# YiyanXu/DiFashion

Measured on AMD Instinct MI355X. Metric: U-Net denoise steps/sec, 4-item outfit @ 64x64x4 latent, higher is better.
Workload: dtype bf16; 1 GPU; BASELINE configs[1]: one 4-item outfit, CFG on (4 branches) -> U-Net batch 16, DDIM-50 schedule, sd15 shape in_channels=8, 64x64x4 latents, 77 text tokens; one outfit per GPU; unet_batch=16, latent=64x64x4, parallelism=outfit-replicas x1 (no data-path collective)

## Files before the change

difashion_amd/csrc/gemm.h:

```cpp
#pragma once
#include <stdint.h>
#include "dfh_common.h"

enum GemmAct { ACT_NONE = 0, ACT_SILU = 1, ACT_LEAKY = 2, ACT_TANH = 3, ACT_GEGLU = 4 };
enum GemmOut {
  OUT_BF16 = 0,
  OUT_BF16_T = 1,
  OUT_F32 = 2,
  OUT_F32_T = 3,
  OUT_FP8_MX = 4,
};

struct GemmArgs {
  const bf16_t* conv_src; int conv_c; int ntaps;
  int Hin, Win, Hout, Wout, stride, ups;
  int pad0;
  const bf16_t* p_src[2]; int p_c[2]; int nplain;
  const bf16_t* W; int ldw;
  const bf16_t* zero;
  int M, N;
  int ksteps;
  int ksplit;
  int n_major;
  int tm_xm, tm_gm;
// ... 21 lines not shown
  const uint8_t* sx;
  const uint8_t* W; const float* sW;
  int M, N, K;
  const float* bias;
  const bf16_t* resid; int ld_res;
  int act;
  void* out; int ld_out; int out_mode;
  uint8_t* out_sx;
  int rows_per_b;
  float* amax;
  const uint8_t* zero;
};

#ifdef __HIPCC__
DFH_DEVICE float2 ln_row_stats(const GemmArgs& a, int m) {
  if (m >= a.M) return float2{0.f, 1.f};
  float sm = 0.f, sq = 0.f, s2 = 0.f;
  for (int t = 0; t < a.ln_parts; ++t) {
    const float2 r = *(const float2*)(a.ln_stat + ((long)t * a.M + m) * 2);
    sm += r.x; sq = fmaf(r.x, r.x, sq); s2 += r.y;
  }
  const float inv = 1.0f / (float)a.ln_parts;
  const float mean = sm * inv;
  const float m2 = s2 + (float)a.ln_cnt * fmaxf(sq - sm * mean, 0.f);
  const float var = m2 * inv / (float)a.ln_cnt;
  return float2{mean, rsqrtf(var + a.ln_eps)};
}
#endif

namespace dfh {
int gemm_fp8_launch(Fp8GemmArgs a, hipStream_t stream);
int amax_slabs_launch(const bf16_t* x, long bstride, int ld, int cols, const int* row0, const int* nrows, float* out, int nslab, int B,
                      hipStream_t stream);
int quant_rows_fp8_launch(const bf16_t* x, int ldx, uint8_t* q, float* scale, int R, int K, hipStream_t stream);
int layernorm_fp8_launch(const bf16_t* x, const float* gamma, const float* beta, uint8_t* q, float* scale, int M, int C, float eps,
                         hipStream_t stream);
int gemm_launch(GemmArgs a, hipStream_t stream, int force_tile = 0, int force_split = 0, int force_order = -1,
                int* gstat_rows = nullptr,
                int* rowstat_bn = nullptr);
int ln_fold_launch(const bf16_t* W, int ldw, const float* gamma, const float* beta, const float* bias, bf16_t* WF, float* s, float* b,
                   int N, int K, hipStream_t stream);
int wino_weight_launch(const bf16_t* W, int ldw, bf16_t* U, int N, int C, int blocked, hipStream_t stream);
bool wino_blocked(int N, int C);
int wino_input_launch(const bf16_t* g, bf16_t* V, int B, int H, int W, int C, hipStream_t stream);
bool gn_wino_ok(int C0, int C1, int G, int H, int W);
int gn_wino_input_launch(const bf16_t* src0, int C0, const bf16_t* src1, int C1, const float* gamma, const float* beta, float eps, int G,
                         bf16_t* V, int B, int H, int W, hipStream_t stream, const bf16_t* Mprev = nullptr, const float* pbias = nullptr,
                         const float* prowvec = nullptr, int prv_ld = 0, int prv_off = 0);
int wino_output_launch(const bf16_t* Mb, bf16_t* out, const float* bias, const float* rowvec, int rv_ld, int rv_off, const bf16_t* resid,
                       int B, int H, int W, int N, hipStream_t stream);
int wino_gemm_tile(const GemmArgs& a);
int ups_phase_fold_launch(const bf16_t* W, int ldw, bf16_t* WP, int N, int C, hipStream_t stream);
int matvec_bias_launch(const bf16_t* W, int ldw, const float* v, const float* b_add, float* b_out, int N, int K, hipStream_t stream);
bool gemm_out2_ok(GemmArgs a);
bool gemm_ln_consumer_ok(GemmArgs a);
int gemm_pick_split(const GemmArgs& a, int* tile_out);
size_t gemm_partial_floats(const GemmArgs& a);
int gemm_count_ksteps(const GemmArgs& a);
bool gemm_wide_eligible(const GemmArgs& a);
int gemm_wide_pick(const GemmArgs& a);
int gemm_wide_launch(GemmArgs a, hipStream_t stream, int variant = 1);
#ifdef DFH_PROBES
bool gemm_halo_eligible(const GemmArgs& a);
int gemm_halo_launch(GemmArgs a, hipStream_t stream);
int gemm_ws_pick(const GemmArgs& a, int min_tiles);
int gemm_ws_launch(GemmArgs a, hipStream_t stream, int bn);
bool gemm_geglu_rows_ok(const GemmArgs& a);
int gemm_geglu_rows_launch(const GemmArgs& a, hipStream_t stream);
bool gemm_persist_ok(const GemmArgs& a);
int gemm_persist_launch(const GemmArgs& a, hipStream_t stream, int max_wgs = 0);
#endif
}
```

difashion_amd/csrc/gemm.hip:

```cpp
#include "gemm.h"
#include "gemm_kiter.h"
#include "gemm_wide_epilogue.h"
#include "norm.h"
#ifdef DFH_PROBES
#include "token_linear.h"
#endif

#include <algorithm>
#include <cstdlib>
#include <cstring>
#include <string>

namespace {

template <int N> DFH_DEVICE void wait_vmcnt() { asm volatile("s_waitcnt vmcnt(%0)" ::"n"(N) : "memory"); }

template <int BM, int BN, int WM, int WN, int NSTAGE, bool LEAN = false, bool WEPI = false>
__global__ __launch_bounds__(WM* WN * 64, (WM * WN == 8 && BM == 128 && 2 * NSTAGE * (BM + BN) * BK * 2 <= 160 * 1024) ? 4 : (WM * WN == 8 ? 2 : 1))
void gemm_bf16_kernel(const GemmArgs a) {
  constexpr int NWV = WM * WN;
  constexpr int TM = BM / WM, TN = BN / WN;
  constexpr int FM = TM / 16, FN = TN / 16;
  constexpr int PA = BM / 8, PB = BN / 8;
  constexpr int IA = (PA + NWV - 1) / NWV, IB = (PB + NWV - 1) / NWV;
// ... 756 lines not shown
  double kk = (double)a.ntaps * a.conv_c;
  for (int i = 0; i < a.nplain; ++i) kk += a.p_c[i];
  const double w_bytes = (double)a.N * kk * 2.0;
  const double a_bytes = a.ntaps ? (double)(a.M / (a.Hout * a.Wout)) * a.Hin * a.Win * a.conv_c * 2.0 : (double)a.M * kk * 2.0;
  const int ntm = (a.M + bm - 1) / bm, ntn = (a.N + bn - 1) / bn;
  if (w_bytes <= 2.0e6 || ntm < 16) return;
  if (ntn >= 16) { a.tm_gm = 8; return; }
  if (!a.ntaps) return;
  int best = 8; double cost = a_bytes + 8.0 * w_bytes;
  for (int xm = 4; xm >= 2; xm >>= 1) {
    if (ntm % xm || ntn % (8 / xm)) continue;
    const double c = (8.0 / xm) * a_bytes + xm * w_bytes;
    if (c < 0.95 * cost) { cost = c; best = xm; }
  }
  if (best != 8) { a.tm_xm = best; a.tm_gm = 8; }
}

int gemm_big_pick(const GemmArgs& a) {
  static const int mode = [] { const char* e = getenv("DFH_GEMM_BIG"); return e ? atoi(e) : 2; }();
  if (mode == 0) return 0;
  if (a.out_mode != OUT_BF16 || a.act == ACT_GEGLU || a.ln_stat) return 0;
  if (a.N % 320 != 0 || (a.ld_out & 7) || (a.resid && (a.ld_res & 7))) return 0;
  const int ksteps = gemm_count_ksteps(a);
  if (ksteps < 16 && (a.ntaps || mode < 3)) return 0;
  if (a.ntaps == 0 && mode < 2) return 0;
  const long tiles = (long)((a.M + 255) / 256) * (a.N / 320), rem = tiles % 256;
  return (tiles >= 224 && (rem == 0 || rem >= 224 || tiles >= 1024)) ? 1 : 0;
}

int gemm_big_geglu_pick(const GemmArgs& a) {
  static const int mode = [] { const char* e = getenv("DFH_GEMM_BIGG"); return e ? atoi(e) : 1; }();
  if (mode == 0 || a.act != ACT_GEGLU || a.out_mode != OUT_BF16 || a.resid || a.rowvec) return 0;
  if (a.N % 256 != 0 || (a.ld_out & 7)) return 0;
  const long tiles = (long)((a.M + 255) / 256) * (a.N / 256), rem = tiles % 256;
  return (tiles >= 224 && (rem == 0 || rem >= 224 || tiles >= 512)) ? 1 : 0;
}

bool wino_blocked(int N, int C) {
  static const bool off = [] { const char* e = getenv("DFH_W_BLOCKED"); return e && e[0] == '0'; }();
  return !off && N % 160 == 0 && C % 64 == 0;
}

int wino_gemm_tile(const GemmArgs& a) {
  static const int pin = [] { const char* e = getenv("DFH_WINO_TILE"); return e ? atoi(e) : -1; }();
  if (pin >= 0) return pin;
  return 0;
}

static bool batched_big_pick(const GemmArgs& a) {
  static const bool off = [] { const char* e = getenv("DFH_BATCH_BIG"); return e && e[0] == '0'; }();
  if (off || a.nbatch <= 1 || a.M < 512 || a.N % 320 != 0) return false;
  const long tiles = (long)((a.M + 255) / 256) * (a.N / 320) * a.nbatch, rem = tiles % 256;
  return tiles >= 224 && (rem == 0 || rem >= 224 || tiles >= 1024);
}

bool gemm_out2_ok(GemmArgs a) {
  if (a.rows_per_b <= 0) a.rows_per_b = a.M;
  a.ksteps = gemm_count_ksteps(a);
  int tile;
  if (gemm_pick_split(a, &tile) != 1) return false;
  return a.out2 != nullptr && a.n_split > 0 && a.n_split < a.N && a.n_split % kTiles[tile].bn == 0 && a.act != ACT_GEGLU &&
         a.out_mode == OUT_BF16 && !a.resid;
}

bool gemm_ln_consumer_ok(GemmArgs a) {
  if (a.rows_per_b <= 0) a.rows_per_b = a.M;
  a.ksteps = gemm_count_ksteps(a);
  int tile;
  if (gemm_pick_split(a, &tile) != 1) return false;
  if (a.act == ACT_GEGLU && ((a.ld_out & 7) || a.N % 32)) return false;
  return a.ntaps == 0 && a.resid == nullptr && a.rowvec == nullptr;
}

int gemm_launch(GemmArgs a, hipStream_t stream, int force_tile, int force_split, int force_order, int* gstat_rows, int* rowstat_bn) {
  if (gstat_rows) *gstat_rows = 0;
  if (rowstat_bn) *rowstat_bn = 0;
  DFH_REQUIRE(a.M > 0 && a.N > 0, "empty GEMM");
  DFH_REQUIRE(a.N % 4 == 0, "N must be a multiple of 4");
  DFH_REQUIRE(a.ntaps == 0 || a.ntaps == 9 || (a.ntaps == 4 && a.phase2x), "ntaps must be 0 or 9 (4 for the phase planes of an upsample conv)");
  DFH_REQUIRE(a.ntaps + a.nplain >= 1, "no K segment");
  DFH_REQUIRE(a.ntaps == 0 || a.conv_c % 8 == 0, "conv channels must be a multiple of 8");
  for (int i = 0; i < a.nplain; ++i) DFH_REQUIRE(a.p_c[i] % 8 == 0, "segment length must be a multiple of 8");
  DFH_REQUIRE(a.zero != nullptr, "zero page missing");
  if (a.rows_per_b <= 0) a.rows_per_b = a.M;
#ifdef DFH_PROBES
  if (force_tile == 30) {
    if (rowstat_bn && a.rowstat) *rowstat_bn = a.N;
    return token_linear_from_gemm(a, stream);
  }
#endif
  a.ksteps = gemm_count_ksteps(a);
  int tile;
  int split = gemm_pick_split(a, &tile);
  const bool force_deep = force_tile == 10;
  if (force_deep) { tile = kEightWave; force_tile = 0; }
  int force_wide = force_tile > kNumTiles ? force_tile - kNumTiles : 0;
  if (force_wide) force_tile = 0;
  if (force_tile > 0) { DFH_REQUIRE(force_tile <= kNumTiles, "unknown tile variant"); tile = force_tile - 1; }
  if (force_split > 0) split = force_split;
  if (a.act == ACT_GEGLU) {
    DFH_REQUIRE(a.N % 32 == 0 && kTiles[tile].bn != 160 && split == 1,
                "GEGLU needs N % 32 == 0, a 64/128-wide tile and no split-K");
    DFH_REQUIRE(a.out_mode == OUT_BF16 && !a.resid && !a.rowvec, "GEGLU epilogue is bias-only, bf16 out");
  }
  split = std::min(split, a.ksteps);
  a.ksplit = split;
// ... 144 lines not shown
```

difashion_amd/csrc/norm.h:

```cpp
#pragma once
#include "dfh_common.h"
#include <algorithm>

enum { GN_MAX_CHUNKS = 64 };

struct GnArgs {
  const bf16_t* src0; const bf16_t* src1;
  int C0, C1;
  int B, HW, G;
  const float* gamma; const float* beta;
  float eps; int silu;
  bf16_t* out;
  uint8_t* out8; float q_mul;
  float* partial;
  float* stats_out;
  const float* pre; int pre_chunks;
  int C, PL, chunks, pix_per_chunk, apix_per_chunk;
};

struct GnBwdArgs {
  const bf16_t* src0; const bf16_t* src1; int C0, C1;
  const bf16_t* dy;
  int B, HW, G;
  const float* gamma; const float* beta; const float* stats; int silu;
  bf16_t* dx0; bf16_t* dx1; int acc0, acc1;
  float* dgamma; float* dbeta;
  float* partial;
  int C, PL, chunks, pix_per_chunk, apix_per_chunk;
};

struct GnFoldArgs {
  const bf16_t* x; int B, HW, C, G; float eps;
  const float* gamma; const float* beta;
  const float* pre; int pre_chunks;
  float* partial;
  const bf16_t* W; int ldw; int N; const float* bias;
  bf16_t* Wimg;
  float* rv;
};

namespace dfh {
int groupnorm_fold_launch(GnFoldArgs a, hipStream_t stream);
int groupnorm_bwd_launch(GnBwdArgs a, hipStream_t stream);
int layernorm_bwd_launch(const bf16_t* x, const bf16_t* dy, const float* gamma, bf16_t* dx, int accumulate, float* dgamma,
                         float* dbeta, int M, int C, float eps, hipStream_t stream);
int groupnorm_launch(GnArgs a, hipStream_t stream);
int layernorm_launch(const bf16_t* x, const float* gamma, const float* beta, bf16_t* y, int M, int C, float eps,
                     hipStream_t stream);
}
```

difashion_amd/csrc/norm.hip:

```cpp
#include "dfh_common.h"
#include "norm.h"
#include <cstring>
#include <cstdlib>

namespace {

struct GnGeom {
  int C, C0, C1, HW, cpg, C8, PL, chunks, pix_per_chunk;
};

DFH_DEVICE const uint4* gn_src(const GnArgs& a, int b, int p, int o) {
  const int o0 = a.C0 >> 3;
  if (o < o0) return (const uint4*)(a.src0 + ((long)(b * a.HW + p) * a.C0 + o * 8));
  return (const uint4*)(a.src1 + ((long)(b * a.HW + p) * a.C1 + (o - o0) * 8));
}

__global__ __launch_bounds__(512) void gn_stats_kernel(const GnArgs a) {
  extern __shared__ __attribute__((aligned(16))) float red[];
  const int C8 = a.C >> 3;
  const int tid = threadIdx.x;
  const int o = tid % C8, pl = tid / C8;
  const int b = blockIdx.y;
  const int p_begin = blockIdx.x * a.pix_per_chunk;
  const int p_end = min(a.HW, p_begin + a.pix_per_chunk);
// ... 464 lines not shown
    const long units = (long)a.HW * (cpg >> 2);
    const bool one_source_per_group = a.C1 == 0 || a.C0 % cpg == 0;
    static const int small_max = [] { const char* e = getenv("DFH_GN_SMALL_MAX"); return e ? atoi(e) : 16; }();
    if ((cpg & 3) == 0 && units <= 256 * small_max && one_source_per_group && (long)a.B * a.G >= 64) {
      ProfScope ps(PC_GNORM, 0.0, (a.out8 ? 3.0 : 4.0) * a.B * (double)a.HW * a.C, stream);
      const dim3 grid(a.G, a.B);
      census(CK_GN_SMALL);
      if (units <= 256 * 8) hipLaunchKernelGGL(gn_small_kernel<8>, grid, dim3(256), 0, stream, a);
      else if (units <= 256 * 16) hipLaunchKernelGGL(gn_small_kernel<16>, grid, dim3(256), 0, stream, a);
      else hipLaunchKernelGGL(gn_small_kernel<32>, grid, dim3(256), 0, stream, a);
      return check_launch("gn_small_kernel");
    }
  }
  {
    static const bool mid_off = [] { const char* e = getenv("DFH_GN_MID"); return e && e[0] == '0'; }();
    const int cpg = a.C / a.G, upp = cpg >> 2;
    if (!mid_off && !a.out8 && (cpg & 3) == 0 && a.HW <= 256 && a.G % 2 == 0) {
      for (int gq = 4; gq >= 2; gq >>= 1) {
        if (a.G % gq || (long)a.B * (a.G / gq) < 128 || gq * upp > 256) continue;
        const int uppb = gq * upp;
        int threads = 256;
        auto units_at = [&](int t) { return t / uppb < 1 ? 1 << 30 : (a.HW + t / uppb - 1) / (t / uppb); };
        while (threads < 1024 && units_at(threads) > 24) threads *= 2;
        if (threads == 1024 && units_at(1024) > 16) threads = 512;
        const int ppb = threads / uppb;
        if (ppb < 1) continue;
        const int units = (a.HW + ppb - 1) / ppb;
        if (units > 32) continue;
        ProfScope ps(PC_GNORM, 0.0, 4.0 * a.B * (double)a.HW * a.C, stream);
        const dim3 grid(a.G / gq, a.B), block(threads);
        census(CK_GN_MID);
        if (units <= 4) hipLaunchKernelGGL(gn_mid_kernel<4>, grid, block, 0, stream, a, gq, ppb);
        else if (units <= 8) hipLaunchKernelGGL(gn_mid_kernel<8>, grid, block, 0, stream, a, gq, ppb);
        else if (units <= 16) hipLaunchKernelGGL(gn_mid_kernel<16>, grid, block, 0, stream, a, gq, ppb);
        else if (units <= 24) hipLaunchKernelGGL((gn_mid_kernel<24, 512>), grid, block, 0, stream, a, gq, ppb);
        else hipLaunchKernelGGL((gn_mid_kernel<32, 512>), grid, block, 0, stream, a, gq, ppb);
        return check_launch("gn_mid_kernel");
      }
    }
  }
  int block, achunks;
  gn_geometry(a, &block, &achunks);
  DFH_REQUIRE(block <= 512, "block too large (more than 4096 channels)");
  const size_t lds = (size_t)a.PL * a.C * 2 * sizeof(float);
  DFH_REQUIRE(lds <= 64 * 1024, "GroupNorm LDS reduction too large");
  ProfScope ps(PC_GNORM, 0.0, (a.out8 ? 3.0 : 4.0) * a.B * (double)a.HW * a.C, stream);
  census(CK_GN_STATS);
  hipLaunchKernelGGL(gn_stats_kernel, dim3(a.chunks, a.B), dim3(block), lds, stream, a);
  if (int rc = check_launch("gn_stats_kernel")) return rc;
  hipLaunchKernelGGL(gn_apply_kernel, dim3(achunks, a.B), dim3(block), 0, stream, a);
  return check_launch("gn_apply_kernel");
}

int groupnorm_fold_launch(GnFoldArgs f, hipStream_t stream) {
  DFH_REQUIRE(f.x && f.gamma && f.beta && f.W && f.Wimg && f.rv && (f.pre || f.partial), "groupnorm fold: null pointer");
  DFH_REQUIRE(f.C % 8 == 0 && f.G > 0 && f.G <= 64 && f.C % f.G == 0 && f.C <= 4096 && f.ldw % 8 == 0 && f.ldw >= f.C && f.N > 0, "groupnorm fold: bad shape");
  const float* partial = f.pre;
  int chunks = f.pre_chunks;
  if (!partial) {
    GnArgs a; std::memset(&a, 0, sizeof(a));
    a.src0 = f.x; a.C0 = a.C = f.C; a.B = f.B; a.HW = f.HW; a.G = f.G; a.partial = f.partial;
    int block, achunks;
    gn_geometry(a, &block, &achunks);
    DFH_REQUIRE(block <= 512, "block too large (more than 4096 channels)");
    const size_t lds = (size_t)a.PL * a.C * 2 * sizeof(float);
    DFH_REQUIRE(lds <= 64 * 1024, "GroupNorm LDS reduction too large");
    ProfScope ps(PC_GNORM, 0.0, 2.0 * a.B * (double)a.HW * a.C, stream);
    census(CK_GN_STATS);
    hipLaunchKernelGGL(gn_stats_kernel, dim3(a.chunks, a.B), dim3(block), lds, stream, a);
    if (int rc = check_launch("gn_stats_kernel")) return rc;
    partial = f.partial; chunks = a.chunks;
  } else {
    DFH_REQUIRE(chunks > 0 && chunks <= (int)GN_MAX_CHUNKS, "producer statistics: 1..64 chunks");
  }
  ProfScope ps(PC_GNORM, 0.0, (double)f.N * f.C * 2.0 * (1.0 + f.B), stream);
  census(CK_GN_FOLDED);
  hipLaunchKernelGGL(gn_fold_kernel, dim3((f.N + 7) / 8, f.B), dim3(256), 0, stream, f, partial, chunks);
  return check_launch("gn_fold_kernel");
}

int layernorm_launch(const bf16_t* x, const float* gamma, const float* beta, bf16_t* y, int M, int C, float eps,
                     hipStream_t stream) {
  DFH_REQUIRE(C % 8 == 0 && C <= 8 * 64 * 4, "LayerNorm width must be a multiple of 8 and <= 2048");
  const dim3 block(256);
  ProfScope ps(PC_LNORM, 0.0, 4.0 * (double)M * C, stream);
  census(CK_LAYERNORM);
  if (C <= 512) hipLaunchKernelGGL((layernorm_kernel<1, 4>), dim3((M + 15) / 16), block, 0, stream, x, gamma, beta, y, M, C, eps);
  else if (C <= 1024) hipLaunchKernelGGL((layernorm_kernel<2, 2>), dim3((M + 7) / 8), block, 0, stream, x, gamma, beta, y, M, C, eps);
  else hipLaunchKernelGGL((layernorm_kernel<4, 1>), dim3((M + 3) / 4), block, 0, stream, x, gamma, beta, y, M, C, eps);
  return check_launch("layernorm_kernel");
}

}
```

difashion_amd/csrc/unet_model.h:

```cpp
#pragma once
#include <algorithm>
#include <cmath>
#include <cstring>
#include <map>
#include <string>
#include <vector>

#include "../../include/difashion_hip.h"
#include "attention.h"
#include "dfh_common.h"
#include "elementwise.h"
#include "gemm.h"
#include "mlp_fused.h"
#ifdef DFH_PROBES
#include "token_linear.h"
#endif
#include "norm.h"
#include "packtab.h"
#include "bwd_elementwise.h"

namespace dfhm {

struct Mat { size_t off = 0; int N = 0, K = 0; };
struct Vec { size_t off = 0; int N = 0; };

enum PackKind { PK_VEC = 0, PK_MAT = 1, PK_CONV3 = 2 };
struct PackOp {
  int param, kind;
  size_t dst;
  int N, K, ldw, row_off, col_off, geglu, accumulate;
  int cin_pad = 0;
};

struct ParamDesc { std::string name; std::vector<int> shape; };

struct TPackOp { int param, conv; size_t dst; int N, K, ldt, t_row_off, t_col_off, geglu, o_pad; };

struct Mat8 { size_t off = 0, soff = 0, boff = 0; int N = 0, K = 0; bool on = false; };

struct ResL {
  int cin = 0, cout = 0, temb_off = 0; bool shortcut = false;
  Vec n1w, n1b, b1, n2w, n2b, b2; Mat w1, w2;
  std::string pre; Mat w1t, w2t, wst;
  size_t u1 = 0, u2 = 0; bool has_u = false;
};
struct Fold { size_t w = 0, s = 0, b = 0; int N = 0, K = 0; };

struct AttL {
  int C = 0, heads = 0, x_off = 0;
  int idx = 0;
  Fold fqkv, fqk, fv, fq2, fff1;
  Fold fffp;
  size_t mlp_img = 0; bool has_mlp = false;
  size_t tl_pin = 0, tl_o1 = 0, tl_q2 = 0, tl_o2 = 0; bool has_tl = false;
  Vec nw, nb, pinb, l1w, l1b, o1b, l2w, l2b, o2b, l3w, l3b, ff1b, ff2b, poutb;
  Mat pin, qk, v, o1, q2, o2, ff1, ff2, pout;
  std::string pre; Mat pint, qkvt, o1t, q2t, o2t, ff1t, ff2t, poutt;
  Mat8 qk8, v8, q28, ff18;
  Mat8 o18, o28, ff28, pout8, pin8;
  size_t f8a_off = 0; bool f8a = false;
};
struct ConvL {
  Mat w; Vec b; int cin = 0, cout = 0; std::string pre; Mat wt;
  size_t ph = 0; bool has_ph = false;
};

struct Tensor {
  bf16_t* p = nullptr; int H = 0, W = 0, C = 0;
  const float* gst = nullptr; int gst_cpg = 0, gst_chunks = 0;
};
// ... 500 lines not shown
      g.zero = zero; g.partial = partial;
      static const bool pre_off = [] { const char* e = getenv("DFH_GN_PRE"); return e && e[0] == '0'; }();
      float* gst = nullptr;
      const int G = u->cfg.norm_num_groups;
      if (o && bump && !pre_off && (o->H * o->W) % 128 == 0 && o->C % G == 0 &&
          (o->H * o->W) / ((o->H * o->W) % 256 == 0 ? 256 : 128) <= (int)GN_MAX_CHUNKS) {
        gst = (float*)bump->alloc((size_t)Ba * G * ((o->H * o->W) / 128) * 2 * sizeof(float));
        g.gstat = gst; g.gstat_cpg = o->C / G; g.gstat_hw = o->H * o->W;
      }
      if (dry) { partial_need = std::max(partial_need, dfh::gemm_partial_floats(g) * sizeof(float)); return; }
      if (dfh::gemm_partial_floats(g) * sizeof(float) > partial_cap) { dfh::set_error("split-K partial buffer too small"); rc = -1; return; }
      int gst_rows = 0;
      rc = dfh::gemm_launch(g, s, 0, 0, -1, &gst_rows, rs_bn);
      if (o && gst_rows) { o->gst = gst; o->gst_cpg = g.gstat_cpg; o->gst_chunks = g.gstat_hw / gst_rows; }
    }
    static GemmArgs base(int M, int N) {
      GemmArgs g; std::memset(&g, 0, sizeof(g));
      g.M = M; g.N = N; g.rows_per_b = M; g.out_mode = OUT_BF16; g.ld_out = N;
      return g;
    }
    void linear(const bf16_t* x, int M, int K, const Mat& W, const Vec* bias, int act, const bf16_t* resid, void* out,
                int N, int out_mode = OUT_BF16, int ld_out = -1, int rows_per_b = 0, Tensor* o = nullptr, Bump* bump = nullptr,
                float* rowstat = nullptr, int* rs_bn = nullptr) {
      GemmArgs g = base(M, N);
      g.p_src[0] = x; g.p_c[0] = K; g.nplain = 1;
      g.W = w16(W); g.ldw = W.K;
      g.bias = bias ? v32(*bias) : nullptr;
      g.act = act; g.resid = resid; g.ld_res = N;
      g.out = out; g.out_mode = out_mode; g.ld_out = ld_out < 0 ? (act == ACT_GEGLU ? N / 2 : N) : ld_out;
      if (rows_per_b) g.rows_per_b = rows_per_b;
      g.rowstat = rowstat;
      gemm(g, o, bump, rs_bn);
    }
    GemmArgs folded(const bf16_t* x, int M, const Fold& f, const float* st, int st_bn, int act, void* out, int out_mode, int ld_out,
                    int rows_per_b) const {
      GemmArgs g = base(M, f.N);
      g.p_src[0] = x; g.p_c[0] = f.K; g.nplain = 1;
      g.W = u->fold_w() + f.w; g.ldw = f.K;
      g.bias = u->fold_v() + f.b; g.ln_s = u->fold_v() + f.s;
      g.ln_stat = st; g.ln_cnt = st_bn; g.ln_parts = st_bn > 0 ? f.K / st_bn : 0; g.ln_eps = 1e-5f;
      g.act = act; g.out = out; g.out_mode = out_mode; g.ld_out = ld_out < 0 ? (act == ACT_GEGLU ? f.N / 2 : f.N) : ld_out;
      if (rows_per_b) g.rows_per_b = rows_per_b;
      return g;
    }
    void groupnorm(const Tensor& x0, const Tensor* x1, const Vec& w, const Vec& b, float eps, int silu, Tensor& out) {
      if (rc || dry) return;
      GnArgs a; std::memset(&a, 0, sizeof(a));
      a.src0 = x0.p; a.C0 = x0.C; a.src1 = x1 ? x1->p : nullptr; a.C1 = x1 ? x1->C : 0;
      a.B = B; a.HW = x0.H * x0.W; a.G = u->cfg.norm_num_groups;
      a.gamma = v32(w); a.beta = v32(b); a.eps = eps; a.silu = silu; a.out = out.p; a.partial = gn_partial;
      if (!x1 && x0.gst && x0.gst_cpg == x0.C / a.G) { a.pre = x0.gst; a.pre_chunks = x0.gst_chunks; }
      rc = dfh::groupnorm_launch(a, s);
    }
    bool use8(const Mat8& m) const { return u->fp8 && m.on; }
    void layernorm8(const bf16_t* x, const Vec& w, const Vec& b, uint8_t* q, float* sc, int M, int C) {
      if (rc || dry) return;
      rc = dfh::layernorm_fp8_launch(x, v32(w), v32(b), q, sc, M, C, 1e-5f, s);
    }
    void linear8(const uint8_t* q, const float* sc, int M, const Mat8& W, const Vec* bias, int act, void* out, int out_mode = OUT_BF16,
                 int ld_out = -1, int rows_per_b = 0, float* amax = nullptr) {
      if (rc || dry) return;
      Fp8GemmArgs g; std::memset(&g, 0, sizeof(g));
      g.A = q; g.sA = sc; g.W = u->arena8 + W.off; g.sW = (const float*)(u->arena8 + W.soff);
      g.M = M; g.N = W.N; g.K = W.K; g.bias = bias ? v32(*bias) : nullptr; g.act = act;
      g.out = out; g.out_mode = out_mode; g.ld_out = ld_out < 0 ? (act == ACT_GEGLU ? W.N / 2 : W.N) : ld_out;
      g.rows_per_b = rows_per_b; g.zero = (const uint8_t*)zero; g.amax = amax;
      rc = dfh::gemm_fp8_launch(g, s);
    }
    Fp8GemmArgs args8(const uint8_t* A, int M, const Mat8& W, const Vec* bias, void* out) const {
      Fp8GemmArgs g; std::memset(&g, 0, sizeof(g));
      g.A = A; g.W = u->arena8 + W.off; g.sW = (const float*)(u->arena8 + W.soff);
      g.M = M; g.N = W.N; g.K = W.K; g.bias = bias ? v32(*bias) : nullptr;
      g.out = out; g.out_mode = OUT_BF16; g.ld_out = W.N; g.zero = (const uint8_t*)zero;
      return g;
    }
    void gemm8(const Fp8GemmArgs& g) {
      if (rc || dry) return;
      rc = dfh::gemm_fp8_launch(g, s);
    }
    void groupnorm8(const Tensor& x, float eps, uint8_t* q) {
      if (rc || dry) return;
      GnArgs a; std::memset(&a, 0, sizeof(a));
      a.src0 = x.p; a.C0 = x.C; a.B = B; a.HW = x.H * x.W; a.G = u->cfg.norm_num_groups; a.eps = eps; a.partial = gn_partial;
      a.out8 = q; a.q_mul = 448.0f / dfh_unet::GN_Z;
      if (x.gst && x.gst_cpg == x.C / a.G) { a.pre = x.gst; a.pre_chunks = x.gst_chunks; }
      rc = dfh::groupnorm_launch(a, s);
    }
    void attention8(const bf16_t* Q, int ldq, const bf16_t* K, int ldk, const bf16_t* Vt, int ldvt, uint8_t* O8, const float* amax, int C,
                    int heads, int Nq, int Nk, long vt_bstride = 0, const float* f8 = nullptr) {
      if (rc || dry) return;
      AttnArgs a; std::memset(&a, 0, sizeof(a));
      if (f8) { a.f8_rq = f8; a.f8_rk = f8 + C; a.f8_rv = f8 + 2 * C; a.f8_hs = f8 + 3 * C; }
      a.vt_bstride = vt_bstride;
      a.Q = Q; a.ldq = ldq; a.K = K; a.ldk = ldk; a.Vt = Vt; a.ldvt = ldvt; a.O8 = O8; a.o_amax = amax; a.ldo = C;
      a.B = B; a.H = heads; a.D = C / heads; a.Nq = Nq; a.Nk = Nk;
      a.scale = 1.0f / sqrtf((float)a.D);
      rc = dfh::attention_launch(a, s);
    }
    void layernorm(const bf16_t* x, const Vec& w, const Vec& b, bf16_t* y, int M, int C) {
      if (rc || dry) return;
      rc = dfh::layernorm_launch(x, v32(w), v32(b), y, M, C, 1e-5f, s);
    }
    void attention(const bf16_t* Q, int ldq, const bf16_t* K, int ldk, const bf16_t* Vt, int ldvt, bf16_t* O, int C,
                   int heads, int Nq, int Nk, long vt_bstride = 0, const float* f8 = nullptr) {
      if (rc || dry) return;
      AttnArgs a; std::memset(&a, 0, sizeof(a));
// ... 55 lines not shown
    void wino_out(const bf16_t* Mb, const Vec& bias, const float* rowvec, int rv_off, const bf16_t* resid, Tensor& o) {
      if (rc || dry) return;
      rc = dfh::wino_output_launch(Mb, o.p, v32(bias), rowvec, temb_ld, rv_off, resid, B, o.H, o.W, o.C, s);
    }

    Tensor resnet(const Tensor& x0, const Tensor* x1, const ResL& r, const float* temb_all) {
      const int H = x0.H, W = x0.W;
      Tensor out = palloc(H, W, r.cout);
      const size_t mark = temp.off;
      Tensor g1 = talloc(H, W, r.cin);
      Tensor h1 = talloc(H, W, r.cout);
      static const int wino_mode = [] { const char* e = getenv("DFH_WINO"); return e ? atoi(e) : 2; }();
      const bool wino = r.has_u && (dry || u->fold_valid) && ((wino_mode >= 1 && H * W <= 64) || (wino_mode >= 2 && H * W <= wino_max_hw()));
      if (wino) {
        static const bool gn_off = [] { const char* e = getenv("DFH_WINO_GN"); return e && e[0] == '0'; }();
        const int G = u->cfg.norm_num_groups;
        static const bool chain_off = [] { const char* e = getenv("DFH_WINO_CHAIN"); return e && e[0] == '0'; }();
        const bf16_t* V1;
        if (!gn_off && dfh::gn_wino_ok(x0.C, x1 ? x1->C : 0, G, H, W)) V1 = wino_in(x0, x1, &r.n1w, &r.n1b);
        else {
          groupnorm(x0, x1, r.n1w, r.n1b, u->cfg.norm_eps, 1, g1);
          V1 = wino_in(g1, nullptr, nullptr, nullptr);
        }
        const bf16_t* M1 = wino_gemm(V1, H, W, r.cin, r.u1, r.cout);
        const bool gn2 = !gn_off && dfh::gn_wino_ok(r.cout, 0, G, H, W);
        const bool chain = gn2 && !chain_off;
        Tensor g2 = talloc(H, W, r.cout);
        const bf16_t* V2;
        if (chain) V2 = wino_in(h1, nullptr, &r.n2w, &r.n2b, M1, &r.b1, temb_all, r.temb_off);
        else {
          wino_out(M1, r.b1, temb_all, r.temb_off, nullptr, h1);
          if (gn2) V2 = wino_in(h1, nullptr, &r.n2w, &r.n2b);
          else {
            groupnorm(h1, nullptr, r.n2w, r.n2b, u->cfg.norm_eps, 1, g2);
            V2 = wino_in(g2, nullptr, nullptr, nullptr);
          }
        }
        const bf16_t* resid = x0.p;
        if (r.shortcut) {
          Tensor sc = talloc(H, W, r.cout);
          GemmArgs g = base(B * H * W, r.cout);
          g.p_src[0] = x0.p; g.p_c[0] = x0.C; g.nplain = 1;
          if (x1) { g.p_src[1] = x1->p; g.p_c[1] = x1->C; g.nplain = 2; }
          g.W = w16(r.w2) + 9 * r.cout; g.ldw = r.w2.K;
          g.out = sc.p;
          gemm(g);
          resid = sc.p;
        }
        const bf16_t* M2 = wino_gemm(V2, H, W, r.cout, r.u2, r.cout);
        wino_out(M2, r.b2, nullptr, 0, resid, out);
        temp.off = mark;
        return out;
      }
      groupnorm(x0, x1, r.n1w, r.n1b, u->cfg.norm_eps, 1, g1);
      {
        GemmArgs g = base(B * H * W, r.cout);
        g.conv_src = g1.p; g.conv_c = r.cin; g.ntaps = 9;
        g.Hin = H; g.Win = W; g.Hout = H; g.Wout = W; g.stride = 1;
        g.W = w16(r.w1); g.ldw = r.w1.K; g.bias = v32(r.b1);
        g.rowvec = temb_all; g.rv_ld = temb_ld; g.rv_off = r.temb_off; g.rows_per_b = H * W;
        g.out = h1.p;
        gemm(g, &h1, &temp);
      }
      Tensor g2 = talloc(H, W, r.cout);
      groupnorm(h1, nullptr, r.n2w, r.n2b, u->cfg.norm_eps, 1, g2);
      {
        GemmArgs g = base(B * H * W, r.cout);
        g.conv_src = g2.p; g.conv_c = r.cout; g.ntaps = 9;
        g.Hin = H; g.Win = W; g.Hout = H; g.Wout = W; g.stride = 1;
        g.W = w16(r.w2); g.ldw = r.w2.K; g.bias = v32(r.b2);
        if (r.shortcut) {
          g.p_src[0] = x0.p; g.p_c[0] = x0.C; g.nplain = 1;
          if (x1) { g.p_src[1] = x1->p; g.p_c[1] = x1->C; g.nplain = 2; }
        } else {
          g.resid = x0.p; g.ld_res = r.cout;
        }
        g.out = out.p;
        gemm(g, &out, &persist);
      }
      temp.off = mark;
      return out;
    }

    Tensor transformer(const Tensor& x, const AttL& a, const bf16_t* kx, const bf16_t* vxt, int T, int pre_n = 0) {
      const int H = x.H, W = x.W, C = a.C, N = H * W;
      const int Bfull = B;
      int M = B * N;
      Tensor out = palloc(H, W, C);
      const size_t mark = temp.off;
      static const bool fold_off = [] { const char* e = getenv("DFH_LN_FOLD"); return e && e[0] == '0'; }();
      const bool f8 = use8(a.qk8);
      const bool f8x = f8 && a.pin8.on;
      const bool fold = u->fold_valid && !fold_off && !f8 && !dry;
      const bool pre = pre_n > 0 && !dry && 2 * pre_n <= Bfull;
      if (pre) { B = Bfull - pre_n; M = B * N; }
      float* st = (float*)temp.alloc((size_t)Ba * N * ((C + 63) / 64) * 2 * sizeof(float));
      int bn = 0;
      auto try_folded = [&](std::initializer_list<GemmArgs> gs) {
        if (!fold || bn <= 0 || C % bn) return false;
        for (const GemmArgs& g : gs) if (!dfh::gemm_ln_consumer_ok(g)) return false;
        for (const GemmArgs& g : gs) gemm(g);
        dfh::census(dfh::CK_LN_FOLDED);
        return true;
      };
#ifdef DFH_PROBES
      static const bool tl_on = [] { const char* e = getenv("DFH_TOKEN_LINEAR"); return e && e[0] == '1'; }();
      const bool tl = fold && tl_on && a.has_tl && dfh::token_linear_eligible(C, C, M);
      auto token_linear = [&](const bf16_t* xin, size_t img, const float* bias, const bf16_t* resid, const Fold* f, bf16_t* o, bool stats) {
        if (rc) return;
        TokLinArgs t; std::memset(&t, 0, sizeof(t));
        t.x = xin; t.img = (const unsigned char*)(u->fold_w() + img); t.bias = bias; t.resid = resid; t.out = o; t.M = M;
        if (f) { t.ln_stat = st; t.ln_parts = C / bn; t.ln_cnt = bn; t.ln_eps = 1e-5f; t.ln_s = u->fold_v() + f->s; t.bias = u->fold_v() + f->b; }
        if (stats) t.rowstat = st;
        rc = dfh::token_linear_launch(t, s);
        if (stats) bn = C;
      };
#else
      constexpr bool tl = false;
      auto token_linear = [](const bf16_t*, size_t, const float*, const bf16_t*, const Fold*, bf16_t*, bool) {};
#endif
      Tensor h0 = talloc(H, W, C);
      uint8_t* a8 = f8x ? (uint8_t*)temp.alloc((size_t)Ba * N * C) : nullptr;
      float* am_self = f8x ? amax_self + (size_t)a.idx * Ba : nullptr;
      const float* am_cross = f8x ? amax_cross + (size_t)a.idx * Ba : nullptr;
      if (f8x) {
        groupnorm8(x, 1e-6f, a8);
        Fp8GemmArgs g = args8(a8, M, a.pin8, nullptr, h0.p);
        g.bias = (const float*)(u->arena8 + a.pin8.boff); g.sa_mul = dfh_unet::GN_Z / 448.0f;
        gemm8(g);
      } else {
        static const int gn_fold_max = [] { const char* e = getenv("DFH_GN_FOLD"); return e ? atoi(e) : 320; }();
// ... 386 lines not shown
```

Measured before the change: 63.00 steps/s.

## Fuse GroupNorm-SiLU apply into the 3x3 conv GEMM halo loader

Adds a conv_gn kernel that reads raw activations into an LDS halo, applies the GroupNorm scale/shift and SiLU on the fly, and runs the implicit-GEMM 3x3 conv with MFMA. Only a stats kernel runs beforehand, so the normalized activation tensor is never written to or re-read from global memory. By default it is used in resnet blocks where the regular GEMM would pick the big tile at 64 or 32 spatial width. The cost is recomputing the normalization for every halo load and a hand-written pipeline with less tuning than the existing GEMM.

After: 63.18 steps/s (median of 6 runs). No clear change (+0.3%).

```diff
diff --git a/difashion_amd/csrc/conv_gn.h b/difashion_amd/csrc/conv_gn.h
--- /dev/null
+++ b/difashion_amd/csrc/conv_gn.h
@@ -0,0 +1,15 @@
+#pragma once
+#include "gemm.h"
+
+struct ConvGnArgs {
+  GemmArgs g;
+  const bf16_t* src1; int C0, C1;
+  const float* gamma; const float* beta;
+  float eps; int G;
+  const float* part; int chunks; int wide_red;
+};
+
+namespace dfh {
+bool conv_gn_ok(const GemmArgs& g, int C0, int C1, int G);
+int conv_gn_launch(ConvGnArgs c, hipStream_t stream, int* gstat_rows);
+}
diff --git a/difashion_amd/csrc/conv_gn.hip b/difashion_amd/csrc/conv_gn.hip
--- /dev/null
+++ b/difashion_amd/csrc/conv_gn.hip
@@ -0,0 +1,279 @@
+#include "conv_gn.h"
+#include "gemm_wide_epilogue.h"
+#include "norm.h"
+
+#include <algorithm>
+
+namespace {
+
+constexpr int CG_BK = 64, CG_BN = 320, CG_NWV = 8;
+constexpr int CG_STATIC = 64 * 4 * 2 + 64 * 8 * 8;
+constexpr int CG_LDS_MAX = 160 * 1024 - CG_STATIC;
+
+template <int IW> constexpr int cg_halo_bytes() { return 6 * (IW + 2) * 128; }
+template <int IW> constexpr int cg_lds_fixed() { return cg_halo_bytes<IW>() + 2 * CG_BN * 128; }
+
+template <int N> DFH_DEVICE void cg_vmcnt() { asm volatile("s_waitcnt vmcnt(%0)" ::"n"(N) : "memory"); }
+
+template <int IW>
+__global__ __launch_bounds__(512, 2) void conv_gn_kernel(const ConvGnArgs c) {
+  constexpr int BM = 4 * IW, BN = CG_BN, WN = 4, NWV = CG_NWV;
+  constexpr int TM = BM / 2, TN = BN / WN;
+  constexpr int FM = TM / 16, FN = TN / 16;
+  constexpr int HWP = IW + 2, HPIX = 6 * HWP;
+  constexpr int HALO = cg_halo_bytes<IW>();
+  constexpr int HE = (HPIX + 63) / 64;
+  constexpr int PB = BN / 8, IB = PB / NWV;
+  constexpr int BSTAGE = BN * 128;
+  constexpr int HW = IW * IW;
+  static_assert(PB % NWV == 0 && TM == 2 * IW && FM * 16 == TM && FN * 16 == TN, "tile");
+
+  extern __shared__ __attribute__((aligned(16))) unsigned char smem[];
+  __shared__ float mean_s[64], rstd_s[64];
+  __shared__ float2 run_s[64][8];
+  float2* sct = (float2*)(smem + HALO + 2 * BSTAGE);
+
+  const GemmArgs& a = c.g;
+  const int tid = threadIdx.x, lane = tid & 63;
+  const int wave = __builtin_amdgcn_readfirstlane(tid >> 6);
+  const int wm = wave / WN, wn = wave % WN;
+  const int ntn = a.N / BN, ntm = a.M / BM;
+  int mt_, nt_;
+  tile_coords(blockIdx.x, ntm, ntn, a.n_major, a.tm_xm, a.tm_gm, mt_, nt_);
+  const int m0 = mt_ * BM, n0 = nt_ * BN;
+  const int bimg = m0 / HW, y0 = (m0 - bimg * HW) / IW;
+  const int C = c.C0 + c.C1;
+  const int nbc = C / CG_BK;
+  const int pc0 = a.nplain > 0 ? a.p_c[0] : 0, pc1 = a.nplain > 1 ? a.p_c[1] : 0;
+  const int nblk = nbc + (pc0 + pc1) / CG_BK, nk = 9 * nbc + (pc0 + pc1) / CG_BK;
+
+  auto glds = [&](const bf16_t* src, unsigned char* dst) {
+    __builtin_amdgcn_global_load_lds((const __attribute__((address_space(1))) void*)src,
+                                     (__attribute__((address_space(3))) void*)dst, 16, 0, 0);
+  };
+  const int srow = lane >> 3;
+  const int sslot = (lane & 7) ^ (((wave & 1) << 2) | (lane >> 4));
+  const unsigned lo_w = (unsigned)(n0 + wave * 8 + srow) * (unsigned)a.ldw + (unsigned)sslot * 8u;
+  const unsigned w_piece = (unsigned)(NWV * 8) * (unsigned)a.ldw;
+  const bf16_t* Wb = a.W;
+  asm volatile("" : "+s"(Wb));
+  auto issue_w = [&](int t, int buf) {
+    unsigned wc;
+    if (t < 9 * nbc) { const int kb = t / 9, tap = t - kb * 9; wc = (unsigned)(tap * C + kb * CG_BK); }
+    else wc = (unsigned)(9 * C + (t - 9 * nbc) * CG_BK);
+    unsigned char* Bs = smem + HALO + buf * BSTAGE + wave * 1024;
+#pragma unroll
+    for (int i = 0; i < IB; ++i) glds(Wb + (lo_w + (wc + (unsigned)i * w_piece)), Bs + i * NWV * 1024);
+  };
+
+  const int hp0 = tid >> 3, hslot = tid & 7;
+  const unsigned hswz = (unsigned)((hslot ^ ((hp0 >> 1) & 7)) << 4);
+  uint4 raw[HE];
+  unsigned vmask = 0;
+  auto prefetch = [&](int kb) {
+    const bf16_t* base; unsigned stride, coff;
+    if (kb < nbc) {
+      const int ch = kb * CG_BK;
+      if (ch < c.C0) { base = a.conv_src; stride = (unsigned)c.C0; coff = (unsigned)ch; }
+      else { base = c.src1; stride = (unsigned)c.C1; coff = (unsigned)(ch - c.C0); }
+    } else {
+      const int j = (kb - nbc) * CG_BK;
+      if (j < pc0) { base = a.p_src[0]; stride = (unsigned)pc0; coff = (unsigned)j; }
+      else { base = a.p_src[1]; stride = (unsigned)pc1; coff = (unsigned)(j - pc0); }
+    }
+    coff += (unsigned)hslot * 8u;
+    vmask = 0;
+#pragma unroll
+    for (int e = 0; e < HE; ++e) {
+      const int hp = hp0 + 64 * e;
+      const int hy = hp / HWP, hx = hp - hy * HWP;
+      const int y = y0 - 1 + hy, x = hx - 1;
+      const bool ok = hp < HPIX && (unsigned)y < (unsigned)IW && (unsigned)x < (unsigned)IW;
+      const unsigned pix = (unsigned)((bimg * IW + y) * IW + x);
+      raw[e] = *(const uint4*)(ok ? base + (pix * stride + coff) : a.zero);
+      vmask |= ok ? (1u << e) : 0u;
+    }
+  };
+  auto write_halo = [&](int kb) {
+    const bool gn = kb < nbc;
+    const float4* sst = (const float4*)(sct + kb * CG_BK + hslot * 8);
+#pragma unroll
+    for (int e = 0; e < HE; ++e) {
+      const int hp = hp0 + 64 * e;
+      if (hp >= HPIX) continue;
+      uint4 o = make_uint4(0u, 0u, 0u, 0u);
+      if ((vmask >> e) & 1u) {
+        if (gn) {
+          float f[8];
+          unpack8(raw[e], f);
+#pragma unroll
+          for (int q = 0; q < 4; ++q) {
+            const float4 v = sst[q];
+            f[2 * q] = silu_f(f[2 * q] * v.x + v.y);
+            f[2 * q + 1] = silu_f(f[2 * q + 1] * v.z + v.w);
+          }
+          o = pack8(f);
+        } else {
+          o = raw[e];
+        }
+      }
+      *(uint4*)(smem + hp * 128 + hswz) = o;
+    }
+  };
+
+  issue_w(0, 0);
+  prefetch(0);
+  const int G = c.G, cpg = C / G;
+  if (c.wide_red) {
+    if (tid < G * 8) {
+      const int g = tid >> 3, sub = tid & 7;
+      const int per = (c.chunks + 7) >> 3, c0 = sub * per, c1 = min(c.chunks, c0 + per);
+      const float2* src = (const float2*)(c.part + ((long)bimg * G + g) * c.chunks * 2);
+      float ss = 0.f, qq = 0.f;
+      for (int k = c0; k < c1; ++k) { const float2 v = src[k]; ss += v.x; qq += v.y; }
+      run_s[g][sub] = float2{ss, qq};
+    }
+    __syncthreads();
+  }
+  if (tid < G) {
+    float ss = 0.f, qq = 0.f;
+    if (c.wide_red) {
+#pragma unroll
+      for (int sub = 0; sub < 8; ++sub) { ss += run_s[tid][sub].x; qq += run_s[tid][sub].y; }
+    } else {
+      const float2* src = (const float2*)(c.part + ((long)bimg * G + tid) * c.chunks * 2);
+      for (int k = 0; k < c.chunks; ++k) { ss += src[k].x; qq += src[k].y; }
+    }
+    const float n = (float)HW * (float)cpg;
+    const float mean = ss / n;
+    const float var = fmaxf(qq / n - mean * mean, 0.f);
+    mean_s[tid] = mean;
+    rstd_s[tid] = rsqrtf(var + c.eps);
+  }
+  __syncthreads();
+  for (int ch = tid; ch < C; ch += NWV * 64) {
+    const int g = ch / cpg;
+    const float w = c.gamma[ch] * rstd_s[g];
+    sct[ch] = float2{w, c.beta[ch] - mean_s[g] * w};
+  }
+  __syncthreads();
+  cg_vmcnt<0>();
+  write_halo(0);
+
+  f32x4_t acc[FM][FN];
+#pragma unroll
+  for (int i = 0; i < FM; ++i)
+#pragma unroll
+    for (int j = 0; j < FN; ++j) acc[i][j] = f32x4_t{0.f, 0.f, 0.f, 0.f};
+
+  const int fr = lane & 15, fg = lane >> 4;
+  int kb = 0, kfirst = 0, klast = 8;
+  int buf = 0;
+  for (int t = 0; t < nk; ++t) {
+    if (t == kfirst + 1 && kb + 1 < nblk) cg_vmcnt<HE>();
+    else cg_vmcnt<0>();
+    asm volatile("s_waitcnt lgkmcnt(0)" ::: "memory");
+    __builtin_amdgcn_s_barrier();
+    asm volatile("" ::: "memory");
+    if (t + 1 < nk) issue_w(t + 1, buf ^ 1);
+    if (t == kfirst && kb + 1 < nblk) prefetch(kb + 1);
+    asm volatile("" ::: "memory");
+    const int tap = kb < nbc ? t - kfirst : 4;
+    const int toff = (tap / 3) * HWP + (tap - (tap / 3) * 3);
+    const unsigned char* Bs = smem + HALO + buf * BSTAGE;
+#pragma unroll
+    for (int ks = 0; ks < 2; ++ks) {
+      bf16x8_t bfr[FN];
+#pragma unroll
+      for (int j = 0; j < FN; ++j) {
+        const int row = wn * TN + j * 16 + fr;
+        bfr[j] = *(const bf16x8_t*)(Bs + row * 128 + (((ks * 4 + fg) ^ ((row >> 1) & 7)) << 4));
+      }
+#pragma unroll
+      for (int i = 0; i < FM; ++i) {
+        const int hp = (2 * wm + (i * 16) / IW) * HWP + (i * 16) % IW + fr + toff;
+        const bf16x8_t af = *(const bf16x8_t*)(smem + hp * 128 + (((ks * 4 + fg) ^ ((hp >> 1) & 7)) << 4));
+#pragma unroll
+        for (int j = 0; j < FN; ++j) acc[i][j] = __builtin_amdgcn_mfma_f32_16x16x32_bf16(bfr[j], af, acc[i][j], 0, 0, 0);
+      }
+    }
+    if (t == klast) {
+      if (kb + 1 < nblk) {
+        cg_vmcnt<0>();
+        asm volatile("s_waitcnt lgkmcnt(0)" ::: "memory");
+        __builtin_amdgcn_s_barrier();
+        asm volatile("" ::: "memory");
+        write_halo(kb + 1);
+      }
+      ++kb; kfirst = t + 1; klast = kb < nbc ? t + 9 : t + 1;
+    }
+    buf ^= 1;
+  }
+  cg_vmcnt<0>();
+  asm volatile("" ::: "memory");
+  wide_epilogue<BM, BN, WN, cg_lds_fixed<IW>()>(a, acc, smem, tid, wm, wn, fr, fg, m0, n0);
+}
+
+template <int IW>
+int cg_launch(const ConvGnArgs& c, int lds, hipStream_t s) {
+  static bool attr_set = false;
+  if (!attr_set) {
+    (void)hipFuncSetAttribute((const void*)conv_gn_kernel<IW>, hipFuncAttributeMaxDynamicSharedMemorySize, CG_LDS_MAX);
+    attr_set = true;
+  }
+  const int tiles = (c.g.M / (4 * IW)) * (c.g.N / CG_BN);
+  hipLaunchKernelGGL(conv_gn_kernel<IW>, dim3(tiles), dim3(CG_NWV * 64), lds, s, c);
+  return dfh::check_launch("conv_gn_kernel");
+}
+
+}
+
+namespace dfh {
+
+bool conv_gn_ok(const GemmArgs& g, int C0, int C1, int G) {
+  if (g.ntaps != 9 || g.stride != 1 || g.ups || g.pad0 || g.phase2x || g.nbatch > 1 || g.w_img_bs || g.w_blocked) return false;
+  if (g.Hin != g.Win || g.Hout != g.Hin || g.Wout != g.Win || (g.Win != 64 && g.Win != 32)) return false;
+  const int HW = g.Win * g.Win, C = C0 + C1;
+  if (g.M <= 0 || g.M % HW || g.N % CG_BN || g.out_mode != OUT_BF16 || g.act != ACT_NONE) return false;
+  if (g.out2 || g.rowstat || g.ln_stat || g.pre_out || (g.ld_out & 7) || (g.resid && (g.ld_res & 7))) return false;
+  if (C0 <= 0 || C0 % CG_BK || C1 < 0 || C1 % CG_BK || C != g.conv_c || G <= 0 || G > 64 || C % G) return false;
+  if (g.nplain < 0 || g.nplain > 2) return false;
+  int kk = 9 * C, cmax = std::max(C0, C1);
+  for (int i = 0; i < g.nplain; ++i) {
+    if (g.p_c[i] <= 0 || g.p_c[i] % CG_BK) return false;
+    kk += g.p_c[i]; cmax = std::max(cmax, g.p_c[i]);
+  }
+  if (g.ldw < kk) return false;
+  if ((double)g.M * cmax >= 2.0e9 || (double)g.N * g.ldw >= 2.0e9) return false;
+  const int lds = (g.Win == 64 ? cg_lds_fixed<64>() : cg_lds_fixed<32>()) + C * 8;
+  return lds <= CG_LDS_MAX;
+}
+
+int conv_gn_launch(ConvGnArgs c, hipStream_t stream, int* gstat_rows) {
+  if (gstat_rows) *gstat_rows = 0;
+  GemmArgs& a = c.g;
+  DFH_REQUIRE(conv_gn_ok(a, c.C0, c.C1, c.G), "conv_gn: launch shape not supported (conv_gn_ok)");
+  DFH_REQUIRE(a.conv_src && a.W && a.zero && a.out && c.gamma && c.beta && c.part && c.chunks > 0 && (c.C1 == 0 || c.src1),
+              "conv_gn: null pointer");
+  for (int i = 0; i < a.nplain; ++i) DFH_REQUIRE(a.p_src[i] != nullptr, "conv_gn: null shortcut operand");
+  const int C = c.C0 + c.C1, IW = a.Win, HW = IW * IW, BM = 4 * IW;
+  int kk = 9 * C;
+  for (int i = 0; i < a.nplain; ++i) kk += a.p_c[i];
+  a.ksteps = 9 * (C / CG_BK) + (kk - 9 * C) / CG_BK;
+  a.ksplit = 1; a.n_major = 0; a.tm_xm = 0; a.tm_gm = 0;
+  if (a.rows_per_b <= 0) a.rows_per_b = a.M;
+  const bool gst = a.gstat && a.gstat_hw == HW && HW / BM <= (int)GN_MAX_CHUNKS && a.gstat_cpg > 0 && CG_BN % a.gstat_cpg == 0 &&
+                   a.N % a.gstat_cpg == 0;
+  if (!gst) a.gstat = nullptr;
+  else if (gstat_rows) *gstat_rows = BM;
+  const int lds = (IW == 64 ? cg_lds_fixed<64>() : cg_lds_fixed<32>()) + C * 8;
+  const double flops = 2.0 * a.M * a.N * (double)kk;
+  const double bytes = (double)a.M * (kk - 8 * C) * 2.0 + (double)a.N * kk * 2.0 + (double)a.M * a.N * 2.0 * (a.resid ? 2.0 : 1.0);
+  ProfScope ps(PC_CONV3, flops, bytes, stream);
+  const int rc = IW == 64 ? cg_launch<64>(c, lds, stream) : cg_launch<32>(c, lds, stream);
+  census(CK_GEMM_ROW);
+  if (a.gstat) census(CK_GSTAT_WRITTEN);
+  return rc;
+}
+
+}
diff --git a/difashion_amd/csrc/gemm.h b/difashion_amd/csrc/gemm.h
--- a/difashion_amd/csrc/gemm.h
+++ b/difashion_amd/csrc/gemm.h
@@ -97,6 +97,7 @@
 int wino_gemm_tile(const GemmArgs& a);
 int ups_phase_fold_launch(const bf16_t* W, int ldw, bf16_t* WP, int N, int C, hipStream_t stream);
 int matvec_bias_launch(const bf16_t* W, int ldw, const float* v, const float* b_add, float* b_out, int N, int K, hipStream_t stream);
+bool gemm_takes_big_tile(GemmArgs a);
 bool gemm_out2_ok(GemmArgs a);
 bool gemm_ln_consumer_ok(GemmArgs a);
 int gemm_pick_split(const GemmArgs& a, int* tile_out);
diff --git a/difashion_amd/csrc/gemm.hip b/difashion_amd/csrc/gemm.hip
--- a/difashion_amd/csrc/gemm.hip
+++ b/difashion_amd/csrc/gemm.hip
@@ -832,6 +832,16 @@
   if (off || a.nbatch <= 1 || a.M < 512 || a.N % 320 != 0) return false;
   const long tiles = (long)((a.M + 255) / 256) * (a.N / 320) * a.nbatch, rem = tiles % 256;
   return tiles >= 224 && (rem == 0 || rem >= 224 || tiles >= 1024);
+}
+
+bool gemm_takes_big_tile(GemmArgs a) {
+  if (a.rows_per_b <= 0) a.rows_per_b = a.M;
+  a.ksteps = gemm_count_ksteps(a);
+  int tile;
+  const int split = std::min(gemm_pick_split(a, &tile), a.ksteps);
+  const bool wide_ok0 = split == 1 && a.out2 == nullptr && a.out_mode == OUT_BF16 && (a.N & 7) == 0 && (a.ld_out & 7) == 0 &&
+                        (!a.resid || (a.ld_res & 7) == 0);
+  return wide_ok0 && a.act != ACT_GEGLU && !a.ln_stat && a.nbatch <= 1 && !a.w_img_bs && gemm_big_pick(a) != 0;
 }
 
 bool gemm_out2_ok(GemmArgs a) {
diff --git a/difashion_amd/csrc/norm.h b/difashion_amd/csrc/norm.h
--- a/difashion_amd/csrc/norm.h
+++ b/difashion_amd/csrc/norm.h
@@ -45,6 +45,7 @@
 int layernorm_bwd_launch(const bf16_t* x, const bf16_t* dy, const float* gamma, bf16_t* dx, int accumulate, float* dgamma,
                          float* dbeta, int M, int C, float eps, hipStream_t stream);
 int groupnorm_launch(GnArgs a, hipStream_t stream);
+int groupnorm_stats_launch(GnArgs a, hipStream_t stream, const float** part, int* chunks, int* wide_red);
 int layernorm_launch(const bf16_t* x, const float* gamma, const float* beta, bf16_t* y, int M, int C, float eps,
                      hipStream_t stream);
 }
diff --git a/difashion_amd/csrc/norm.hip b/difashion_amd/csrc/norm.hip
--- a/difashion_amd/csrc/norm.hip
+++ b/difashion_amd/csrc/norm.hip
@@ -540,6 +540,30 @@
   return check_launch("gn_apply_kernel");
 }
 
+int groupnorm_stats_launch(GnArgs a, hipStream_t stream, const float** part, int* chunks, int* wide_red) {
+  a.C = a.C0 + a.C1;
+  DFH_REQUIRE(a.C % 8 == 0 && a.C0 % 8 == 0 && a.C1 % 8 == 0 && a.G > 0 && a.G <= 64 && a.C % a.G == 0 && a.C <= 4096,
+              "groupnorm statistics: bad shape");
+  DFH_REQUIRE(a.src0 != nullptr && (a.C1 == 0 || a.src1 != nullptr) && (a.partial != nullptr || a.pre != nullptr),
+              "groupnorm statistics: null pointer");
+  int block, achunks;
+  gn_geometry(a, &block, &achunks);
+  DFH_REQUIRE(block <= 512, "block too large (more than 4096 channels)");
+  *wide_red = block >= a.G * 8 ? 1 : 0;
+  if (a.pre) {
+    DFH_REQUIRE(a.C1 == 0 && a.pre_chunks > 0 && a.pre_chunks <= (int)GN_MAX_CHUNKS, "producer statistics: one source, 1..64 chunks");
+    *part = a.pre; *chunks = a.pre_chunks;
+    return 0;
+  }
+  const size_t lds = (size_t)a.PL * a.C * 2 * sizeof(float);
+  DFH_REQUIRE(lds <= 64 * 1024, "GroupNorm LDS reduction too large");
+  ProfScope ps(PC_GNORM, 0.0, 2.0 * a.B * (double)a.HW * a.C, stream);
+  census(CK_GN_STATS);
+  hipLaunchKernelGGL(gn_stats_kernel, dim3(a.chunks, a.B), dim3(block), lds, stream, a);
+  *part = a.partial; *chunks = a.chunks;
+  return check_launch("gn_stats_kernel");
+}
+
 int groupnorm_fold_launch(GnFoldArgs f, hipStream_t stream) {
   DFH_REQUIRE(f.x && f.gamma && f.beta && f.W && f.Wimg && f.rv && (f.pre || f.partial), "groupnorm fold: null pointer");
   DFH_REQUIRE(f.C % 8 == 0 && f.G > 0 && f.G <= 64 && f.C % f.G == 0 && f.C <= 4096 && f.ldw % 8 == 0 && f.ldw >= f.C && f.N > 0, "groupnorm fold: bad shape");
diff --git a/difashion_amd/csrc/unet_model.h b/difashion_amd/csrc/unet_model.h
--- a/difashion_amd/csrc/unet_model.h
+++ b/difashion_amd/csrc/unet_model.h
@@ -16,6 +16,7 @@
 #include "token_linear.h"
 #endif
 #include "norm.h"
+#include "conv_gn.h"
 #include "packtab.h"
 #include "bwd_elementwise.h"
 
@@ -622,6 +623,37 @@
       if (!x1 && x0.gst && x0.gst_cpg == x0.C / a.G) { a.pre = x0.gst; a.pre_chunks = x0.gst_chunks; }
       rc = dfh::groupnorm_launch(a, s);
     }
+    bool conv_gn_on(const GemmArgs& g, const Tensor& x0, const Tensor* x1) const {
+      static const int mode = [] { const char* e = getenv("DFH_CONV_GN"); return e ? atoi(e) : 64; }();
+      if (mode == 0 || (mode > 1 && g.Win != mode)) return false;
+      if (mode == 64) {
+        GemmArgs p = g; p.zero = zero; p.partial = partial;
+        if (!dfh::gemm_takes_big_tile(p)) return false;
+      }
+      return dfh::conv_gn_ok(g, x0.C, x1 ? x1->C : 0, u->cfg.norm_num_groups);
+    }
+    void conv_gn(GemmArgs g, const Tensor& x0, const Tensor* x1, const Vec& w, const Vec& b, Tensor* o, Bump* bump) {
+      if (rc) return;
+      static const bool pre_off = [] { const char* e = getenv("DFH_GN_PRE"); return e && e[0] == '0'; }();
+      const int G = u->cfg.norm_num_groups;
+      float* gst = nullptr;
+      if (!pre_off && (o->H * o->W) % 128 == 0 && o->C % G == 0 && (o->H * o->W) / 128 <= (int)GN_MAX_CHUNKS) {
+        gst = (float*)bump->alloc((size_t)Ba * G * ((o->H * o->W) / 128) * 2 * sizeof(float));
+        g.gstat = gst; g.gstat_cpg = o->C / G; g.gstat_hw = o->H * o->W;
+      }
+      if (dry) return;
+      g.zero = zero;
+      GnArgs a; std::memset(&a, 0, sizeof(a));
+      a.src0 = x0.p; a.C0 = x0.C; a.src1 = x1 ? x1->p : nullptr; a.C1 = x1 ? x1->C : 0;
+      a.B = B; a.HW = x0.H * x0.W; a.G = G; a.eps = u->cfg.norm_eps; a.silu = 1; a.partial = gn_partial;
+      if (!x1 && x0.gst && x0.gst_cpg == x0.C / G) { a.pre = x0.gst; a.pre_chunks = x0.gst_chunks; }
+      ConvGnArgs c; std::memset(&c, 0, sizeof(c));
+      c.g = g; c.src1 = a.src1; c.C0 = a.C0; c.C1 = a.C1; c.gamma = v32(w); c.beta = v32(b); c.eps = a.eps; c.G = G;
+      if ((rc = dfh::groupnorm_stats_launch(a, s, &c.part, &c.chunks, &c.wide_red))) return;
+      int gst_rows = 0;
+      rc = dfh::conv_gn_launch(c, s, &gst_rows);
+      if (gst_rows) { o->gst = gst; o->gst_cpg = g.gstat_cpg; o->gst_chunks = g.gstat_hw / gst_rows; }
+    }
     bool use8(const Mat8& m) const { return u->fp8 && m.on; }
     void layernorm8(const bf16_t* x, const Vec& w, const Vec& b, uint8_t* q, float* sc, int M, int C) {
       if (rc || dry) return;
@@ -783,21 +815,24 @@
         temp.off = mark;
         return out;
       }
-      groupnorm(x0, x1, r.n1w, r.n1b, u->cfg.norm_eps, 1, g1);
       {
         GemmArgs g = base(B * H * W, r.cout);
-        g.conv_src = g1.p; g.conv_c = r.cin; g.ntaps = 9;
+        g.conv_src = x0.p; g.conv_c = r.cin; g.ntaps = 9;
         g.Hin = H; g.Win = W; g.Hout = H; g.Wout = W; g.stride = 1;
         g.W = w16(r.w1); g.ldw = r.w1.K; g.bias = v32(r.b1);
         g.rowvec = temb_all; g.rv_ld = temb_ld; g.rv_off = r.temb_off; g.rows_per_b = H * W;
         g.out = h1.p;
-        gemm(g, &h1, &temp);
+        if (conv_gn_on(g, x0, x1)) conv_gn(g, x0, x1, r.n1w, r.n1b, &h1, &temp);
+        else {
+          groupnorm(x0, x1, r.n1w, r.n1b, u->cfg.norm_eps, 1, g1);
+          g.conv_src = g1.p;
+          gemm(g, &h1, &temp);
+        }
       }
       Tensor g2 = talloc(H, W, r.cout);
-      groupnorm(h1, nullptr, r.n2w, r.n2b, u->cfg.norm_eps, 1, g2);
       {
         GemmArgs g = base(B * H * W, r.cout);
-        g.conv_src = g2.p; g.conv_c = r.cout; g.ntaps = 9;
+        g.conv_src = h1.p; g.conv_c = r.cout; g.ntaps = 9;
         g.Hin = H; g.Win = W; g.Hout = H; g.Wout = W; g.stride = 1;
         g.W = w16(r.w2); g.ldw = r.w2.K; g.bias = v32(r.b2);
         if (r.shortcut) {
@@ -807,7 +842,12 @@
           g.resid = x0.p; g.ld_res = r.cout;
         }
         g.out = out.p;
-        gemm(g, &out, &persist);
+        if (conv_gn_on(g, h1, nullptr)) conv_gn(g, h1, nullptr, r.n2w, r.n2b, &out, &persist);
+        else {
+          groupnorm(h1, nullptr, r.n2w, r.n2b, u->cfg.norm_eps, 1, g2);
+          g.conv_src = g2.p;
+          gemm(g, &out, &persist);
+        }
       }
       temp.off = mark;
       return out;
```
